# flashlight/wav2letter

Measured on AMD Instinct MI355X. Metric: utterances/sec, higher is better.
Workload: dtype f32

## Files before the change

### include/w2l_hip.h

```cpp
#ifndef W2L_HIP_H_
#define W2L_HIP_H_

#include <stddef.h>
#include <stdint.h>

#ifdef __cplusplus
extern "C" {
#endif

typedef void* w2l_stream_t;

typedef enum {
  W2L_OK = 0,
  W2L_EINVAL = 1,
  W2L_EHIP = 2,
  W2L_EUNSUPPORTED = 3
} w2l_status;

typedef enum {
  W2L_SCALE_NONE = 0,
  W2L_SCALE_INPUT_SZ = 1,
  W2L_SCALE_INPUT_SZ_SQRT = 2,
  W2L_SCALE_TARGET_SZ = 3,
  W2L_SCALE_TARGET_SZ_SQRT = 4
// ... 142 lines not shown
                                    float* dx, w2l_stream_t stream);
int w2l_tds_conv_bf16_backward_filter(const w2l_conv_desc* d, const float* x, const float* dy, float* dw, w2l_stream_t stream);
int w2l_tds_conv_bf16_backward_filter_bias(const w2l_conv_desc* d, const float* x, const float* dy, float* dw, float* dbias,
                                           w2l_stream_t stream);

typedef struct {
  uint16_t* rowMajor;
  size_t ldRows;
  uint16_t* transposed;
  size_t ldTrans;
} w2l_bf16_image_sink;
int w2l_gemm_bf16_images(int M, int N, int K, const uint16_t* A, int lda, const uint16_t* B, int ldb, float* C, int ldc,
                         const float* bias, int relu, const w2l_gemm_epilogue* epilogue, const w2l_bf16_image_sink* images,
                         const uint16_t* maskImage, size_t ldMask, float maskScale, w2l_stream_t stream);
size_t w2l_layernorm_scratch_doubles(int groups, size_t inner);
int w2l_residual_layernorm_forward(int groups, size_t inner, float* a, const float* x, float* r,
                                   float* y, const float* gammaBeta, float eps, double p,
                                   uint32_t seed, uint32_t rngStream, double* stats,
                                   float* meanRstd, w2l_stream_t stream);
int w2l_layernorm_backward(int groups, size_t inner, const float* r, const float* dy,
                           const float* gammaBeta, const float* meanRstd, float* dr,
                           float* dGammaBeta, const float* maskSrc, float* dmask, float maskScale,
                           double* sums, w2l_stream_t stream);
int w2l_residual_layernorm_forward_images(int groups, size_t inner, float* a, const float* x, float* r, float* y,
                                          const float* gammaBeta, float eps, double p, uint32_t seed, uint32_t rngStream,
                                          float* meanRstd, const w2l_bf16_image_sink* yImages, w2l_stream_t stream);
int w2l_layernorm_backward_images(int groups, size_t inner, const float* r, const float* dy, const float* gammaBeta,
                                  const float* meanRstd, float* dr, float* dGammaBeta, const float* maskSrc, float* dmask,
                                  float maskScale, double* sums, const w2l_bf16_image_sink* drImages, double imageDropP,
                                  uint32_t imageDropSeed, uint32_t imageDropStream, w2l_stream_t stream);
int w2l_dropout_inplace(float* x, size_t n, double p, uint32_t seed, uint32_t rngStream,
                        w2l_stream_t stream);
int w2l_dropout_copy(float* y, const float* x, size_t n, double p, uint32_t seed, uint32_t rngStream,
                     w2l_stream_t stream);
int w2l_mask_backward(const float* dy, const float* src, float* dx, size_t n, float scale,
                      w2l_stream_t stream);

int w2l_hexpand_forward(const float* x, float* xe, size_t rows, int H, int C, int kh, int padh, w2l_stream_t stream);
int w2l_hexpand_backward(const float* dxe, float* dx, size_t rows, int H, int C, int kh, int padh, w2l_stream_t stream);
typedef struct {
  int M, N, K, G1, G2;
  long long sam, sak, a1, a2;
  long long sbk, sbn, b1, b2;
  long long ldc, c1, c2;
  int accumulate;
  int bandMode, bandT, bandH, bandOff;
// ... 115 lines not shown
```

### wav2letter_amd/_lib.py

```python
import ctypes as C
import os

_HERE = os.path.dirname(os.path.abspath(__file__))
SO_PATH = os.environ.get("W2L_HIP_SO") or os.path.join(_HERE, "libw2l_hip.so")
_lib = None

W2L_OK, W2L_EINVAL, W2L_EHIP, W2L_EUNSUPPORTED = 0, 1, 2, 3
_ERR = {1: "W2L_EINVAL (bad shape / null pointer)", 2: "W2L_EHIP (HIP runtime error)",
        3: "W2L_EUNSUPPORTED (shape outside this build)"}


class W2LError(RuntimeError):
    pass


class W2LInvalidArgument(W2LError, ValueError):
    """mirrors the std::invalid_argument Flashlight's criteria throw"""


def _load(path):
    if not os.path.exists(path):
        raise W2LError(
            f"{path} not found: build it with `python -c 'import __graft_entry__ as g; g.build()'` "
            "or `make -C wav2letter_amd/csrc` (no CPU fallback exists)")
# ... 88 lines not shown
    w2l_gemm_bf16_ex = (_i, [_i, _i, _i, _p, _i, _i, _p, _i, _i, _p, _i, _p, _i, _p, _p])
    w2l_gemm_bf16_grouped = (_i, [_i, _i, _i, _i, _p, _i, _p, _i, _p, _i, _p, _p])
    w2l_tds_conv_bf16_image_elems = (_sz, [_p])
    w2l_tds_conv_bf16_prepare = (_i, [_p, _p, _p, _p, _p])
    w2l_tds_conv_bf16_forward = (_i, [_p, _p, _p, _p, _p, _i, _p])
    w2l_tds_conv_bf16_backward_data = (_i, [_p, _p, _p, _p, _p, _p])
    w2l_tds_conv_bf16_backward_filter = (_i, [_p, _p, _p, _p, _p])
    w2l_tds_conv_bf16_backward_filter_bias = (_i, [_p, _p, _p, _p, _p, _p])
    w2l_mfsc_spectrum = (_i, [_p, _p, _sz, _i, _i, _i, _p])
    w2l_mfsc_log_transpose = (_i, [_p, _p, _i, _i, _i, _i, _f, _p])
    w2l_weightnorm_forward = (_i, [_p, _p, _p, _p, _i, _i, _p])
    w2l_weightnorm_backward = (_i, [_p, _p, _p, _p, _p, _p, _p, _i, _i, _p])
    w2l_conv_out_len = (_i, [_i, _i, _i, _i, _i])
    w2l_conv_same_pad = (_i, [_i, _i, _i])
    w2l_conv_forward = (_i, [_p, _p, _p, _p, _p, _i, _p])
    w2l_conv_backward_data = (_i, [_p, _p, _p, _p, _i, _p])
    w2l_conv_backward_data_add = (_i, [_p, _p, _p, _p, _p, _p])
    w2l_conv_backward_filter = (_i, [_p, _p, _p, _p, _p, _p])
    w2l_layernorm_scratch_doubles = (_sz, [_i, _sz])
    w2l_residual_layernorm_forward_images = (_i, [_i, _sz, _p, _p, _p, _p, _p, _f, _d, _u32, _u32, _p, _p, _p])
    w2l_layernorm_backward_images = (_i, [_i, _sz, _p, _p, _p, _p, _p, _p, _p, _p, _f, _p, _p, _d, _u32, _u32, _p])
    w2l_residual_layernorm_forward = (_i, [_i, _sz, _p, _p, _p, _p, _p, _f, _d, _u32, _u32, _p, _p, _p])
    w2l_layernorm_backward = (_i, [_i, _sz, _p, _p, _p, _p, _p, _p, _p, _p, _f, _p, _p])
    w2l_dropout_inplace = (_i, [_p, _sz, _d, _u32, _u32, _p])
    w2l_dropout_copy = (_i, [_p, _p, _sz, _d, _u32, _u32, _p])
    w2l_linear_forward_dropout = (_i, [_i, _i, _i, _p, _p, _p, _p, _i, _d, _u32, _u32, _p])
    w2l_linear_forward_dropout_add = (_i, [_i, _i, _i, _p, _p, _p, _p, _p, _i, _d, _u32, _u32, _p])
    w2l_linear_backward_data_add = (_i, [_i, _i, _i, _p, _p, _p, _p, _p])
    w2l_mask_backward = (_i, [_p, _p, _p, _sz, _f, _p])
    w2l_hexpand_forward = (_i, [_p, _p, _sz, _i, _i, _i, _i, _p])
    w2l_hexpand_backward = (_i, [_p, _p, _sz, _i, _i, _i, _i, _p])
    w2l_bgemm_f32 = (_i, [_p, _p, _p, _p, _p])
    w2l_bgemm_bf16 = (_i, [_p, _p, _p, _p, _p])
    w2l_attn_softmax_forward = (_i, [_p, _p, _p, _i, _i, _i, _i, _i, _i, _i, _f, _p])
    w2l_attn_fused_forward = (_i, [_p, _p, _p, _p, _p, _p, _p, _p, _p, _p])
    w2l_attn_fused_backward_workspace = (_sz, [_p, _i])
    w2l_attn_fused_forward_images = (_i, [_p, _p, _p, _p, _p, _p, _p, _p, _p, _p, _p])
    w2l_attn_fused_backward_images = (_i, [_p, _p, _p, _p, _p, _p, _p, _p, _p, _p, _p, _p, _p, _p, _p, _sz, _p])
    w2l_attn_fused_backward = (_i, [_p, _p, _p, _p, _p, _p, _p, _p, _p, _p, _p, _p, _sz, _p])
    w2l_attn_key_lengths = (_i, [_p, _i, _i, _i, _p, _p])
    w2l_attn_key_lengths_full = (_i, [_p, _p, _i, _i, _i, _p, _p])
    w2l_attn_softmax_backward = (_i, [_p, _p, _p, _i, _i, _i, _i, _i, _i, _i, _f, _p])
    w2l_pool_time_forward = (_i, [_p, _p, _i, _i, _i, _i, _i, _p])
    w2l_pool_time_backward = (_i, [_p, _p, _p, _i, _i, _i, _i, _i, _p])
    w2l_axpy = (_i, [_p, _p, _sz, _f, _p])
    w2l_transpose = (_i, [_p, _p, _i, _i, _i, _p])
# ... 62 lines not shown
```

### wav2letter_amd/csrc/elementwise.hip

```cpp
#include "common.hpp"
#include "gemm.hpp"

namespace w2l {

constexpr int kEwThreads = 256;

static inline unsigned ew_grid(size_t n4) {
  size_t g = (n4 + kEwThreads - 1) / kEwThreads;
  if (g > 256 * 16) g = 256 * 16;
  if (g < 1) g = 1;
  return (unsigned)g;
}

constexpr int kLnMaxParts = 64;
constexpr size_t kLnSmall = 8192;

__device__ __forceinline__ void block_partial2(double a, double b, double* part) {
  __shared__ double sm[2][kEwThreads / 64];
#pragma unroll
  for (int off = 32; off > 0; off >>= 1) {
    a += __shfl_xor(a, off);
    b += __shfl_xor(b, off);
  }
  const int w = threadIdx.x >> 6;
  if ((threadIdx.x & 63) == 0) { sm[0][w] = a; sm[1][w] = b; }
  __syncthreads();
  if (threadIdx.x == 0) {
    double sa = 0, sb = 0;
#pragma unroll
    for (int i = 0; i < kEwThreads / 64; ++i) { sa += sm[0][i]; sb += sm[1][i]; }
    part[0] = sa;
    part[1] = sb;
  }
}
__device__ __forceinline__ void sum_parts(const double* __restrict__ part, int g, int nparts, double& a, double& b) {
  a = 0; b = 0;
  for (int i = 0; i < nparts; ++i) { a += part[2 * ((size_t)g * nparts + i)]; b += part[2 * ((size_t)g * nparts + i) + 1]; }
}

__global__ __launch_bounds__(kEwThreads) void residual_dropout_stats_k(
    float* __restrict__ a, const float* __restrict__ x, float* __restrict__ r, double* __restrict__ part,
    size_t inner, uint32_t thr, float keepScale, uint32_t seed, uint32_t stream) {
  const int g = blockIdx.y;
  const size_t base = (size_t)g * inner;
  const size_t n4 = inner >> 2;
  double s = 0, ss = 0;
  for (size_t i = (size_t)blockIdx.x * blockDim.x + threadIdx.x; i < n4; i += (size_t)gridDim.x * blockDim.x) {
    const size_t e = base + 4 * i;
    float4 av = *(const float4*)(a + e);
    float4 rv = x ? *(const float4*)(x + e) : make_float4(0.f, 0.f, 0.f, 0.f);
    if (thr) {
      av.x = keep_elem(e, seed, stream, thr) ? av.x * keepScale : 0.f;
      av.y = keep_elem(e + 1, seed, stream, thr) ? av.y * keepScale : 0.f;
      av.z = keep_elem(e + 2, seed, stream, thr) ? av.z * keepScale : 0.f;
      av.w = keep_elem(e + 3, seed, stream, thr) ? av.w * keepScale : 0.f;
      if (r != a || !x) *(float4*)(a + e) = av;
    }
    rv.x += av.x; rv.y += av.y; rv.z += av.z; rv.w += av.w;
    if (r != a || x) *(float4*)(r + e) = rv;
    const float p1 = (rv.x + rv.y) + (rv.z + rv.w);
    const float p2 = (rv.x * rv.x + rv.y * rv.y) + (rv.z * rv.z + rv.w * rv.w);
    s += (double)p1;
    ss += (double)p2;
  }
  block_partial2(s, ss, part + 2 * ((size_t)g * gridDim.x + blockIdx.x));
}

__global__ __launch_bounds__(kEwThreads) void ln_apply_k(const float* __restrict__ r, float* __restrict__ y,
                                                        const double* __restrict__ part,
                                                        float* __restrict__ meanRstd, size_t inner,
                                                        const float* __restrict__ gammaBeta, float eps) {
  const int g = blockIdx.y;
  double s1, s2;
  sum_parts(part, g, gridDim.x, s1, s2);
  const double mu = s1 / (double)inner;
  double var = s2 / (double)inner - mu * mu;
  if (var < 0) var = 0;
  const float rstd = (float)(1.0 / sqrt(var + (double)eps));
  const float muf = (float)mu;
  if (blockIdx.x == 0 && threadIdx.x == 0) { meanRstd[2 * g] = muf; meanRstd[2 * g + 1] = rstd; }
// ... 164 lines not shown
  if (threadIdx.x == 0) { meanRstd[2 * g] = muf; meanRstd[2 * g + 1] = rstd; }
  const float gam = gammaBeta[0] * rstd, bet = gammaBeta[1];
  for (size_t i = threadIdx.x; i < inner; i += kEwThreads) y[base + i] = (r[base + i] - muf) * gam + bet;
}

__global__ __launch_bounds__(kEwThreads) void ln_bwd_reduce_k(const float* __restrict__ r,
                                                             const float* __restrict__ dy,
                                                             const float* __restrict__ meanRstd,
                                                             double* __restrict__ part, size_t inner) {
  const int g = blockIdx.y;
  const float mu = meanRstd[2 * g], rstd = meanRstd[2 * g + 1];
  const size_t base = (size_t)g * inner, n4 = inner >> 2;
  double s1 = 0, s2 = 0;
  for (size_t i = (size_t)blockIdx.x * blockDim.x + threadIdx.x; i < n4; i += (size_t)gridDim.x * blockDim.x) {
    float4 rv = *(const float4*)(r + base + 4 * i);
    float4 dv = *(const float4*)(dy + base + 4 * i);
    s1 += (double)((dv.x + dv.y) + (dv.z + dv.w));
    s2 += (double)((dv.x * ((rv.x - mu) * rstd) + dv.y * ((rv.y - mu) * rstd)) +
                   (dv.z * ((rv.z - mu) * rstd) + dv.w * ((rv.w - mu) * rstd)));
  }
  block_partial2(s1, s2, part + 2 * ((size_t)g * gridDim.x + blockIdx.x));
}

__global__ __launch_bounds__(kEwThreads) void ln_bwd_apply_k(const float* __restrict__ r,
                                                            const float* __restrict__ dy,
                                                            const float* __restrict__ meanRstd,
                                                            const double* __restrict__ part,
                                                            double* __restrict__ sums,
                                                            const float* __restrict__ gammaBeta,
                                                            float* __restrict__ dr,
                                                            const float* __restrict__ maskSrc,
                                                            float* __restrict__ dmask, float maskScale,
                                                            size_t inner) {
  const int g = blockIdx.y;
  const float mu = meanRstd[2 * g], rstd = meanRstd[2 * g + 1];
  double S1, S2;
  sum_parts(part, g, gridDim.x, S1, S2);
  if (blockIdx.x == 0 && threadIdx.x == 0) { sums[2 * g] = S1; sums[2 * g + 1] = S2; }
  const float c1 = (float)(S1 / (double)inner), c2 = (float)(S2 / (double)inner);
  const float gr = gammaBeta[0] * rstd;
  const size_t base = (size_t)g * inner, n4 = inner >> 2;
  for (size_t i = (size_t)blockIdx.x * blockDim.x + threadIdx.x; i < n4; i += (size_t)gridDim.x * blockDim.x) {
    const size_t e = base + 4 * i;
    float4 rv = *(const float4*)(r + e);
    float4 dv = *(const float4*)(dy + e);
    float4 o;
    o.x = gr * (dv.x - c1 - (rv.x - mu) * rstd * c2);
    o.y = gr * (dv.y - c1 - (rv.y - mu) * rstd * c2);
    o.z = gr * (dv.z - c1 - (rv.z - mu) * rstd * c2);
    o.w = gr * (dv.w - c1 - (rv.w - mu) * rstd * c2);
    *(float4*)(dr + e) = o;
    if (dmask) {
      float4 mv = *(const float4*)(maskSrc + e);
      float4 d2;
      d2.x = mv.x > 0.f ? o.x * maskScale : 0.f;
      d2.y = mv.y > 0.f ? o.y * maskScale : 0.f;
      d2.z = mv.z > 0.f ? o.z * maskScale : 0.f;
      d2.w = mv.w > 0.f ? o.w * maskScale : 0.f;
      *(float4*)(dmask + e) = d2;
    }
  }
}

template <int NJ>
__global__ __launch_bounds__(kEwThreads) void ln_bwd_small_k(const float* __restrict__ r, const float* __restrict__ dy,
                                                            const float* __restrict__ meanRstd,
                                                            double* __restrict__ sums,
                                                            const float* __restrict__ gammaBeta,
                                                            float* __restrict__ dr,
                                                            const float* __restrict__ maskSrc,
                                                            float* __restrict__ dmask, float maskScale,
                                                            size_t inner) {
  __shared__ double bc[2];
  const int g = blockIdx.x;
  const float mu = meanRstd[2 * g], rstd = meanRstd[2 * g + 1];
  const size_t base = (size_t)g * inner;
  const int n4 = (int)(inner >> 2);
  float4 xh[NJ], dv[NJ], mvs[NJ];
  const int lastc = n4 - 1;
#pragma unroll
  for (int j = 0; j < NJ; ++j) {
// ... 424 lines not shown
    }
#undef W2L_LN_FWDW
    W2L_LAUNCH_CHECK();
    return W2L_OK;
  }
  if (inner <= kLnSmall) {
    const int nj = (int)((inner / 4 + kEwThreads - 1) / kEwThreads);
#define W2L_LN_FWD(NJ_)                                                                                                     \
  case NJ_:                                                                                                                 \
    hipLaunchKernelGGL(residual_ln_small_k<NJ_>, dim3((unsigned)groups), dim3(kEwThreads), 0, W2L_S, a, x, r, y, meanRstd,  \
                       inner, gammaBeta, eps, thr, ks, seed, rngStream);                                                    \
    break
    switch (nj) {
      W2L_LN_FWD(1); W2L_LN_FWD(2); W2L_LN_FWD(3); W2L_LN_FWD(4); W2L_LN_FWD(5); W2L_LN_FWD(6); W2L_LN_FWD(7);
      default: hipLaunchKernelGGL(residual_ln_small_k<kLnSmallV>, dim3((unsigned)groups), dim3(kEwThreads), 0, W2L_S, a, x, r, y, meanRstd,
                                  inner, gammaBeta, eps, thr, ks, seed, rngStream);
    }
#undef W2L_LN_FWD
    W2L_LAUNCH_CHECK();
    return W2L_OK;
  }
  double* part = stats + 2 * (size_t)groups;
  dim3 grid(ln_parts(inner), (unsigned)groups);
  hipLaunchKernelGGL(residual_dropout_stats_k, grid, dim3(kEwThreads), 0, W2L_S, a, x, r, part, inner, thr, ks, seed, rngStream);
  W2L_LAUNCH_CHECK();
  hipLaunchKernelGGL(ln_apply_k, grid, dim3(kEwThreads), 0, W2L_S, r, y, part, meanRstd, inner, gammaBeta, eps);
  W2L_LAUNCH_CHECK();
  return W2L_OK;
}

W2L_API int w2l_layernorm_backward(int groups, size_t inner, const float* r, const float* dy,
                                   const float* gammaBeta, const float* meanRstd, float* dr,
                                   float* dGammaBeta, const float* maskSrc, float* dmask, float maskScale,
                                   double* sums, w2l_stream_t stream) {
  if (groups <= 0 || inner == 0 || (inner & 3) || !r || !dy || !gammaBeta || !meanRstd || !dr || !sums)
    return W2L_EINVAL;
  if (inner / 4 <= 64 * (size_t)kLnWaveV && ln_wave_enabled()) {
    const int nj = (int)((inner / 4 + 63) / 64);
    const dim3 grid((unsigned)((groups + kEwThreads / 64 - 1) / (kEwThreads / 64)));
#define W2L_LN_BWDW(NJ_)                                                                                                 \
  case NJ_:                                                                                                              \
    hipLaunchKernelGGL(ln_bwd_wave_k<NJ_>, grid, dim3(kEwThreads), 0, W2L_S, groups, r, dy, meanRstd, sums, gammaBeta,   \
                       dr, maskSrc, maskSrc ? dmask : nullptr, maskScale, inner);                                        \
    break
    switch (nj) {
      W2L_LN_BWDW(1); W2L_LN_BWDW(2); W2L_LN_BWDW(3); W2L_LN_BWDW(4); W2L_LN_BWDW(5); W2L_LN_BWDW(6); W2L_LN_BWDW(7); W2L_LN_BWDW(8);
      default: hipLaunchKernelGGL(ln_bwd_wave_k<kLnWaveV>, grid, dim3(kEwThreads), 0, W2L_S, groups, r, dy, meanRstd, sums, gammaBeta,
                                  dr, maskSrc, maskSrc ? dmask : nullptr, maskScale, inner);
    }
#undef W2L_LN_BWDW
    W2L_LAUNCH_CHECK();
  } else if (inner <= kLnSmall) {
    const int nj = (int)((inner / 4 + kEwThreads - 1) / kEwThreads);
#define W2L_LN_BWD(NJ_)                                                                                                  \
  case NJ_:                                                                                                              \
    hipLaunchKernelGGL(ln_bwd_small_k<NJ_>, dim3((unsigned)groups), dim3(kEwThreads), 0, W2L_S, r, dy, meanRstd, sums,   \
                       gammaBeta, dr, maskSrc, maskSrc ? dmask : nullptr, maskScale, inner);                             \
    break
    switch (nj) {
      W2L_LN_BWD(1); W2L_LN_BWD(2); W2L_LN_BWD(3); W2L_LN_BWD(4); W2L_LN_BWD(5); W2L_LN_BWD(6); W2L_LN_BWD(7);
      default: hipLaunchKernelGGL(ln_bwd_small_k<kLnSmallV>, dim3((unsigned)groups), dim3(kEwThreads), 0, W2L_S, r, dy, meanRstd, sums,
                                  gammaBeta, dr, maskSrc, maskSrc ? dmask : nullptr, maskScale, inner);
    }
#undef W2L_LN_BWD
    W2L_LAUNCH_CHECK();
  } else {
    double* part = sums + 2 * (size_t)groups;
    dim3 grid(ln_parts(inner), (unsigned)groups);
    hipLaunchKernelGGL(ln_bwd_reduce_k, grid, dim3(kEwThreads), 0, W2L_S, r, dy, meanRstd, part, inner);
    W2L_LAUNCH_CHECK();
    hipLaunchKernelGGL(ln_bwd_apply_k, grid, dim3(kEwThreads), 0, W2L_S, r, dy, meanRstd, part, sums, gammaBeta, dr,
                       maskSrc, maskSrc ? dmask : nullptr, maskScale, inner);
    W2L_LAUNCH_CHECK();
  }
  if (dGammaBeta) {
    hipLaunchKernelGGL(ln_param_grad_k, dim3(1), dim3(1024), 0, W2L_S, sums, groups, dGammaBeta);
    W2L_LAUNCH_CHECK();
  }
  return W2L_OK;
}

__global__ __launch_bounds__(kEwThreads) void dropout_copy_k(float* __restrict__ y, const float* __restrict__ x, size_t n,
                                                            uint32_t thr, float keepScale, uint32_t seed, uint32_t stream) {
  const size_t n4 = n >> 2;
  for (size_t i = (size_t)blockIdx.x * blockDim.x + threadIdx.x; i < n4; i += (size_t)gridDim.x * blockDim.x) {
    const size_t e = 4 * i;
    float4 v = *(const float4*)(x + e);
    v.x = keep_elem(e, seed, stream, thr) ? v.x * keepScale : 0.f;
    v.y = keep_elem(e + 1, seed, stream, thr) ? v.y * keepScale : 0.f;
    v.z = keep_elem(e + 2, seed, stream, thr) ? v.z * keepScale : 0.f;
    v.w = keep_elem(e + 3, seed, stream, thr) ? v.w * keepScale : 0.f;
    *(float4*)(y + e) = v;
  }
  for (size_t e = (n4 << 2) + (size_t)blockIdx.x * blockDim.x + threadIdx.x; e < n; e += (size_t)gridDim.x * blockDim.x)
    y[e] = keep_elem(e, seed, stream, thr) ? x[e] * keepScale : 0.f;
}

W2L_API int w2l_dropout_copy(float* y, const float* x, size_t n, double p, uint32_t seed, uint32_t rngStream,
                             w2l_stream_t stream) {
  if (!x || !y || ((((uintptr_t)x) | ((uintptr_t)y)) & 15)) return W2L_EINVAL;
  const uint32_t thr = dropout_threshold(p);
  if (!n) return W2L_OK;
// ... 172 lines not shown
```

### wav2letter_amd/csrc/host/net.cpp

```cpp
#include <algorithm>
#include <cmath>
#include <cstring>
#include <sstream>

#include "w2l_host.hpp"

namespace w2l {

std::string Act::str() const {
  std::ostringstream os;
  os << "(";
  for (int i = 0; i < 4; ++i) {
    os << (i ? "," : "");
    if (d[i].f.size() == 1 && d[i].f[0].kind == F_TIME) os << "T";
    else if (d[i].f.size() == 1 && d[i].f[0].kind == F_BATCH) os << "B";
    else os << d[i].size();
  }
  os << ") phys[" << B << "][" << T << "][" << F << "]";
  return os.str();
}

static constexpr int kSymT = 1000003, kSymB = 1000033;

Act actInput(int B, int T, int nFeat) {
// ... 349 lines not shown
    if (!rides) check(w2l_colsum(g, b.g(cx), (size_t)M, bl.out, cx.stream), "bwd b");
  }
  void backward(Ctx& cx, float* ar, const float* x, const BfImage& xImg, const float* dy, const BfImage& dyImg, const float* addend, float* dx, double p) {
    const bool mixed = cx.bf16;
    const bool rides2 = mixed ? lin2BiasRides(cx) : biasWithWeight, rides1 = mixed ? bl1.biasRides(xImg, w1->g(cx), b1->g(cx)) : biasWithWeight;
    const float sc = (float)(1.0 / (1.0 - p));
    float *u = ar + uOff, *du = ar + duOff;
    weightGrad(cx, ar, bl2, u, uImg, dy, dyImg, *w2, *b2, rides2);
    if (!mixed) {
      check(w2l_linear_backward_data(M, hidden, in, dy, w2->w(cx), du, 0, u, sc, cx.stream), "lin2 bwd x");
    } else if (!(uOnlyImages && bl2.backwardDataImages(cx, ar, dyImg, rides1 ? nullptr : du, &duImg, uImg, sc))) {
      if (uOnlyImages) throw std::runtime_error(tag("u was kept as images only, but the image-writing backward-data product refused"));
      bl2.backwardData(cx, ar, dyImg, du, u, sc, nullptr, 0);
      duImg.convert(cx, ar, du, tag("du images").c_str());
    }
    weightGrad(cx, ar, bl1, x, xImg, du, duImg, *w1, *b1, rides1);
    if (mixed) bl1.backwardData(cx, ar, duImg, dx, nullptr, 1.f, addend, 0);
    else check(w2l_linear_backward_data_add(M, in, hidden, du, w1->w(cx), addend, dx, cx.stream), "lin1 bwd x");
  }
};

constexpr size_t kLnImageElems = (size_t)1 << 22;
static bool lnForward(Ctx& cx, float* ar, int groups, size_t inner, float* a, const float* x, float* r, float* y, const float* gb, double p,
                      uint32_t seed, uint32_t stream, double* stats, float* mr, const BfImage* img, const char* what) {
  if (img && img->rows == groups && (size_t)img->cols == inner && (size_t)groups * inner <= kLnImageElems) {
    const w2l_bf16_image_sink k = img->sink(cx, ar);
    const int st = w2l_residual_layernorm_forward_images(groups, inner, a, x, r, y, gb, 1e-5f, p, seed, stream, mr, &k, cx.stream);
    if (st == W2L_OK) return true;
    if (st != W2L_EUNSUPPORTED) w2lCheck(st, what);
  }
  w2lCheck(w2l_residual_layernorm_forward(groups, inner, a, x, r, y, gb, 1e-5f, p, seed, stream, stats, mr, cx.stream), what);
  return false;
}
static bool lnBackward(Ctx& cx, float* ar, int groups, size_t inner, const float* r, const float* dy, const float* gb, const float* mr, float* dr,
                       float* dgb, const float* maskSrc, float* dmask, float maskScale, double* sums, const BfImage* img, double imgP,
                       uint32_t imgSeed, uint32_t imgStream, const char* what) {
  if (img && img->rows == groups && (size_t)img->cols == inner && (size_t)groups * inner <= kLnImageElems) {
    const w2l_bf16_image_sink k = img->sink(cx, ar);
    const int st = w2l_layernorm_backward_images(groups, inner, r, dy, gb, mr, dr, dgb, maskSrc, dmask, maskScale, sums, &k, imgP, imgSeed,
                                                 imgStream, cx.stream);
    if (st == W2L_OK) return true;
    if (st != W2L_EUNSUPPORTED) w2lCheck(st, what);
  }
  w2lCheck(w2l_layernorm_backward(groups, inner, r, dy, gb, mr, dr, dgb, maskSrc, dmask, maskScale, sums, cx.stream), what);
  return false;
}

struct WNState {
  bool on = false;
  P v, g;
  size_t wOff = 0, dwOff = 0, normOff = 0, dotOff = 0;
  int K = 0, N = 0;
};

// ... 313 lines not shown
    w2lCheck(w2l_glu_forward(x, y, M, half, c.stream), "glu fwd");
  }
  void backward(Ctx& c, float* arena, const float* dy, float*& dx, bool) override {
    dx = arena + dxOff;
    w2lCheck(w2l_glu_backward(xSaved, dy, dx, M, half, c.stream), "glu bwd");
  }
};

class TDSLayer : public Layer {
 public:
  int c, kw, h, l, l2, rPad;
  double p;
  bool lnTime;
  P wc, bc, gb1, w1, b1, w2, b2, gb2;
  w2l_conv_desc d{};
  int B = 0, T = 0, M = 0, groups = 0;
  size_t inner = 0, n = 0;
  size_t aOff, r1Off, y1Off, vOff, outOff, st1Off, mr1Off, st2Off, mr2Off;
  size_t dsOff, dy1Off, dr1Off, daOff, dxOff;
  const float* xSaved = nullptr;
  FeedForward ff;
  BfImage y1Img, dvImg;
  size_t convImgElems = 0, convImgFOff = 0, convImgBOff = 0;

  std::string name() const override { return "TDSBlock"; }
  void registerParams(std::vector<ParamInfo>& t) override {
    ParamInfo q;
    q = ParamInfo(); q.name = "tds.conv.w"; q.numel = (size_t)kw * c * c; q.refShape = {kw, 1, c, c}; q.kind = 1;
    q.kw = kw; q.cin = c; q.cout = c; q.initBound = std::sqrt(1.0 / ((double)c * kw)); addParam(t, q, wc);
    q = ParamInfo(); q.name = "tds.conv.b"; q.numel = c; q.refShape = {1, 1, c, 1}; q.initBound = std::sqrt(1.0 / ((double)c * kw)); addParam(t, q, bc);
    q = ParamInfo(); q.name = "tds.ln1.weight+bias"; q.numel = 2; q.refShape = {1}; q.kind = 3; addParam(t, q, gb1);
    q = ParamInfo(); q.name = "tds.lin1.w"; q.numel = (size_t)l * l2; q.refShape = {l2, l}; q.kind = 2; q.cin = l; q.cout = l2;
    q.initBound = std::sqrt(1.0 / (double)l); addParam(t, q, w1);
    q = ParamInfo(); q.name = "tds.lin1.b"; q.numel = l2; q.refShape = {l2}; q.initBound = std::sqrt(1.0 / (double)l); addParam(t, q, b1);
    q = ParamInfo(); q.name = "tds.lin2.w"; q.numel = (size_t)l2 * l; q.refShape = {l, l2}; q.kind = 2; q.cin = l2; q.cout = l;
    q.initBound = std::sqrt(1.0 / (double)l2); addParam(t, q, w2);
    q = ParamInfo(); q.name = "tds.lin2.b"; q.numel = l; q.refShape = {l}; q.initBound = std::sqrt(1.0 / (double)l2); addParam(t, q, b2);
    q = ParamInfo(); q.name = "tds.ln2.weight+bias"; q.numel = 2; q.refShape = {1}; q.kind = 3; addParam(t, q, gb2);
  }
  Act plan(const Act& in, Planner& pl) override {
    int H;
    requireConvLayout(in, c, "TDSBlock", H);
    if (H != h) throw std::invalid_argument("TDSBlock: expected H=" + std::to_string(h) + ", input " + in.str());
    int pL, pR;
    if (rPad < 0) { pL = pR = samePad(in.T, kw, 1); }
    else { if (rPad > kw - 1) throw std::invalid_argument("TDSBlock: invalid right padding"); pR = rPad; pL = kw - 1 - rPad; }
    d = {in.B, in.T, h, c, c, kw, 1, pL, pR};
    if (w2l_conv_out_len(in.T, kw, 1, pL, pR) != in.T) throw std::invalid_argument("TDSBlock: conv must preserve T (odd kw)");
    B = in.B; T = in.T; M = B * T; n = in.numel();
    groups = lnTime ? B : B * T;
    inner = n / groups;
    if (inner % 4) throw std::invalid_argument("TDSBlock: LayerNorm size must be a multiple of 4");
    aOff = pl.alloc(n); r1Off = pl.alloc(n); y1Off = pl.alloc(n); vOff = pl.alloc(n); outOff = pl.alloc(n);
    st1Off = pl.alloc(2 * w2l_layernorm_scratch_doubles(groups, inner)); mr1Off = pl.alloc(2 * (size_t)groups);
    st2Off = pl.alloc(2 * w2l_layernorm_scratch_doubles(groups, inner)); mr2Off = pl.alloc(2 * (size_t)groups);
    dsOff = pl.alloc(n); dy1Off = pl.alloc(n); dr1Off = pl.alloc(n); daOff = pl.alloc(n); dxOff = pl.alloc(n);
    ff.joinInLin2 = l2 % 32 == 0;
    ff.biasWithWeight = true;
    ff.plan(pl, "tds", M, l, l2, w1, b1, w2, b2);
    y1Img.plan(pl, M, l, true); dvImg.plan(pl, M, l);
    convImgElems = h % 16 == 0 ? w2l_tds_conv_bf16_image_elems(&d) : 0;
    if (convImgElems) { convImgFOff = pl.allocBf16(convImgElems); convImgBOff = pl.allocBf16(convImgElems); }
    return in;
  }
  void forward(Ctx& cx, float* ar, const float* x, float*& y) override {
    hipStream_t s = cx.stream;
    const double pd = cx.train ? p : 0.0;
    xSaved = x;
    float *a = ar + aOff, *r1 = ar + r1Off, *y1 = ar + y1Off, *v = ar + vOff, *out = ar + outOff;
    if (cx.bf16 && convImgElems) {
      w2lCheck(w2l_tds_conv_bf16_prepare(&d, wc.w(cx), bfp(ar, convImgFOff), bfp(ar, convImgBOff), s), "tds conv images");
      w2lCheck(w2l_tds_conv_bf16_forward(&d, x, bfp(ar, convImgFOff), bc.w(cx), a, 1, s), "tds conv bf16");
    } else {
      w2lCheck(w2l_conv_forward(&d, x, wc.w(cx), bc.w(cx), a, 1, s), "tds conv");
    }
    const bool y1Images = lnForward(cx, ar, groups, inner, a, x, r1, y1, gb1.w(cx), pd, cx.seed, rngStream, (double*)(ar + st1Off), ar + mr1Off,
                                    cx.bf16 ? &y1Img : nullptr, "tds ln1");
    if (cx.bf16) {
      const w2l_bf16_convert_desc wd[3] = {y1Img.desc(ar, y1), ff.bl1.w.desc(ar, w1.w(cx)), ff.bl2.w.desc(ar, w2.w(cx))};
      w2lCheck(w2l_bf16_convert_multi(y1Images ? 2 : 3, wd + (y1Images ? 1 : 0), s), "tds y1 + weight images");
      if (!y1Images) y1Img.ensureOnes(cx, ar);
    }
    const bool joined = ff.forward(cx, ar, y1, y1Img, v, pd, rngStream + 1);
    w2lCheck(w2l_residual_layernorm_forward(groups, inner, v, joined ? nullptr : y1, v, out, gb2.w(cx), 1e-5f, joined ? 0.0 : pd,
                                            joined ? 0 : cx.seed, joined ? 0 : rngStream + 2, (double*)(ar + st2Off), ar + mr2Off, s), "tds ln2");
    y = out;
  }
  void backward(Ctx& cx, float* ar, const float* dy, float*& dx, bool needDx) override {
    hipStream_t s = cx.stream;
    const double pd = cx.train ? p : 0.0;
    const float sc = (float)(1.0 / (1.0 - pd));
    float *a = ar + aOff, *y1 = ar + y1Off, *v = ar + vOff;
    float *ds = ar + dsOff, *dy1 = ar + dy1Off, *dr1 = ar + dr1Off, *da = ar + daOff;
    const bool rides2 = cx.bf16 && ff.lin2BiasRides(cx);
    const bool maskInConvert = pd > 0 && rides2;
    const bool dvImages = lnBackward(cx, ar, groups, inner, v, dy, gb2.w(cx), ar + mr2Off, ds, gb2.g(cx), nullptr, nullptr, 1.f,
                                     (double*)(ar + st2Off), cx.bf16 && (pd == 0 || maskInConvert) ? &dvImg : nullptr, pd, cx.seed,
                                     rngStream + 2, "tds ln2 bwd");
    const float* dv = ds;
    if (pd > 0 && !maskInConvert) {
      w2lCheck(w2l_dropout_copy(dy1, ds, n, pd, cx.seed, rngStream + 2, s), "tds do2 bwd");
      dv = dy1;
    }
    if (cx.bf16 && !dvImages) {
      if (maskInConvert) dvImg.convertDropout(cx, ar, ds, pd, cx.seed, rngStream + 2, "tds dv images (masked)");
      else dvImg.convert(cx, ar, dv, "tds dv images");
    }
    ff.backward(cx, ar, y1, y1Img, dv, dvImg, ds, dy1, pd);
    w2lCheck(w2l_layernorm_backward(groups, inner, ar + r1Off, dy1, gb1.w(cx), ar + mr1Off, dr1, gb1.g(cx), a, da, sc,
                                    (double*)(ar + st1Off), s), "tds ln1 bwd");
    if (cx.bf16 && convImgElems) {
      w2lCheck(w2l_tds_conv_bf16_backward_filter_bias(&d, xSaved, da, wc.g(cx), bc.g(cx), s), "tds conv bwd filter + bias bf16");
      if (needDx) {
        dx = ar + dxOff;
        w2lCheck(w2l_tds_conv_bf16_backward_data(&d, da, bfp(ar, convImgBOff), dr1, dx, s), "tds conv bwd data bf16");
      }
      return;
    }
    w2lCheck(w2l_conv_backward_filter(&d, xSaved, da, wc.g(cx), bc.g(cx), s), "tds conv bwd filter");
    if (needDx) {
      dx = ar + dxOff;
      w2lCheck(w2l_conv_backward_data_add(&d, da, wc.w(cx), dr1, dx, s), "tds conv bwd data");
    }
  }
};

class PoolTimeLayer : public Layer {
 public:
  int w = 1, stride = 1;
  int B = 0, T = 0, To = 0, F = 0;
  size_t yOff = 0, dxOff = 0;
  const float* xSaved = nullptr;
  std::string name() const override { return "Pool2D"; }
// ... 673 lines not shown
```

### wav2letter_amd/ops.py

```python
import ctypes as C

import torch

from . import _lib
from ._lib import ConvDesc, check


def _s():
    return torch.cuda.current_stream().cuda_stream


def _p(t):
    return t.data_ptr() if t is not None else None


def gemm(A, B, a_kcontig=True, b_kcontig=False, bias=None, relu=False, splitk=1):
    M, K = (A.shape if a_kcontig else A.shape[::-1])
    N = B.shape[0] if b_kcontig else B.shape[1]
    Cm = torch.empty(M, N, device=A.device, dtype=torch.float32)
    check(_lib.lib().w2l_gemm_f32(M, N, K, _p(A), A.stride(0), int(a_kcontig), _p(B), B.stride(0), int(b_kcontig),
                                  _p(Cm), N, _p(bias), int(relu), splitk, _s()), "gemm")
    return Cm


# ... 70 lines not shown
def _ln_scratch(groups, inner):
    return int(_lib.lib().w2l_layernorm_scratch_doubles(groups, inner))


def residual_layernorm_forward(a, x, gamma_beta, groups, eps=1e-5, p=0.0, seed=0, stream_id=0):
    inner = a.numel() // groups
    r = torch.empty_like(a)
    y = torch.empty_like(a)
    stats = torch.empty(_ln_scratch(groups, inner), device=a.device, dtype=torch.float64)
    mr = torch.empty(2 * groups, device=a.device, dtype=torch.float32)
    check(_lib.lib().w2l_residual_layernorm_forward(groups, inner, _p(a), _p(x), _p(r), _p(y), _p(gamma_beta), eps,
                                                    p, seed, stream_id, _p(stats), _p(mr), _s()), "res_ln_fwd")
    return y, r, mr


def layernorm_backward(r, dy, gamma_beta, mean_rstd, groups, mask_src=None, mask_scale=1.0):
    inner = r.numel() // groups
    dr = torch.empty_like(r)
    dgb = torch.empty(2, device=r.device, dtype=torch.float32)
    dmask = torch.empty_like(r) if mask_src is not None else None
    sums = torch.empty(_ln_scratch(groups, inner), device=r.device, dtype=torch.float64)
    check(_lib.lib().w2l_layernorm_backward(groups, inner, _p(r), _p(dy), _p(gamma_beta), _p(mean_rstd), _p(dr),
                                            _p(dgb), _p(mask_src), _p(dmask), mask_scale, _p(sums), _s()), "ln_bwd")
    return dr, dgb, dmask


def linear_forward_dropout(x, w, bias, relu, p, seed, stream_id):
    M, K = x.shape
    N = w.shape[1]
    y = torch.empty(M, N, device=x.device, dtype=torch.float32)
    check(_lib.lib().w2l_linear_forward_dropout(M, K, N, _p(x), _p(w), _p(bias), _p(y), int(relu), p, seed, stream_id, _s()), "linear_forward_dropout")
    return y


def linear_forward_dropout_add(x, w, bias, add, relu, p, seed, stream_id):
    M, K = x.shape
    N = w.shape[1]
    y = torch.empty(M, N, device=x.device, dtype=torch.float32)
    check(_lib.lib().w2l_linear_forward_dropout_add(M, K, N, _p(x), _p(w), _p(bias), _p(add), _p(y), int(relu), p, seed, stream_id, _s()),
          "linear_forward_dropout_add")
    return y


def linear_backward_data_add(dy, w, add):
    M, N = dy.shape
    K = w.shape[0]
# ... 154 lines not shown
```

Measured before the change: 328.6.

## Fuse dropout mask bits and recomputed dropout into TDS layernorm backward

```diff
diff --git a/include/w2l_hip.h b/include/w2l_hip.h
--- a/include/w2l_hip.h
+++ b/include/w2l_hip.h
@@ -188,6 +188,16 @@
                            const float* gammaBeta, const float* meanRstd, float* dr,
                            float* dGammaBeta, const float* maskSrc, float* dmask, float maskScale,
                            double* sums, w2l_stream_t stream);
+size_t w2l_layernorm_mask_bytes(int groups, size_t inner);
+int w2l_residual_layernorm_forward_mask(int groups, size_t inner, const float* a, const float* x, float* r, float* y,
+                                        const float* gammaBeta, float eps, double p, uint32_t seed, uint32_t rngStream,
+                                        double* stats, float* meanRstd, uint8_t* mask, w2l_stream_t stream);
+int w2l_layernorm_backward_mask(int groups, size_t inner, const float* r, const float* dy, const float* gammaBeta,
+                                const float* meanRstd, float* dr, float* dGammaBeta, const uint8_t* mask, float* dmask,
+                                float maskScale, double* sums, w2l_stream_t stream);
+int w2l_layernorm_backward_dropout(int groups, size_t inner, const float* r, const float* dy, const float* gammaBeta,
+                                   const float* meanRstd, float* dr, float* dGammaBeta, float* dmask, double p, uint32_t seed,
+                                   uint32_t rngStream, double* sums, w2l_stream_t stream);
 int w2l_residual_layernorm_forward_images(int groups, size_t inner, float* a, const float* x, float* r, float* y,
                                           const float* gammaBeta, float eps, double p, uint32_t seed, uint32_t rngStream,
                                           float* meanRstd, const w2l_bf16_image_sink* yImages, w2l_stream_t stream);
diff --git a/wav2letter_amd/_lib.py b/wav2letter_amd/_lib.py
--- a/wav2letter_amd/_lib.py
+++ b/wav2letter_amd/_lib.py
@@ -134,6 +134,10 @@
     w2l_layernorm_backward_images = (_i, [_i, _sz, _p, _p, _p, _p, _p, _p, _p, _p, _f, _p, _p, _d, _u32, _u32, _p])
     w2l_residual_layernorm_forward = (_i, [_i, _sz, _p, _p, _p, _p, _p, _f, _d, _u32, _u32, _p, _p, _p])
     w2l_layernorm_backward = (_i, [_i, _sz, _p, _p, _p, _p, _p, _p, _p, _p, _f, _p, _p])
+    w2l_layernorm_mask_bytes = (_sz, [_i, _sz])
+    w2l_residual_layernorm_forward_mask = (_i, [_i, _sz, _p, _p, _p, _p, _p, _f, _d, _u32, _u32, _p, _p, _p, _p])
+    w2l_layernorm_backward_mask = (_i, [_i, _sz, _p, _p, _p, _p, _p, _p, _p, _p, _f, _p, _p])
+    w2l_layernorm_backward_dropout = (_i, [_i, _sz, _p, _p, _p, _p, _p, _p, _p, _d, _u32, _u32, _p, _p])
     w2l_dropout_inplace = (_i, [_p, _sz, _d, _u32, _u32, _p])
     w2l_dropout_copy = (_i, [_p, _p, _sz, _d, _u32, _u32, _p])
     w2l_linear_forward_dropout = (_i, [_i, _i, _i, _p, _p, _p, _p, _i, _d, _u32, _u32, _p])
diff --git a/wav2letter_amd/csrc/elementwise.hip b/wav2letter_amd/csrc/elementwise.hip
--- a/wav2letter_amd/csrc/elementwise.hip
+++ b/wav2letter_amd/csrc/elementwise.hip
@@ -1,3 +1,4 @@
+#include <type_traits>
 #include "common.hpp"
 #include "gemm.hpp"
 
@@ -38,9 +39,11 @@
   for (int i = 0; i < nparts; ++i) { a += part[2 * ((size_t)g * nparts + i)]; b += part[2 * ((size_t)g * nparts + i) + 1]; }
 }
 
+template <bool MASK>
 __global__ __launch_bounds__(kEwThreads) void residual_dropout_stats_k(
-    float* __restrict__ a, const float* __restrict__ x, float* __restrict__ r, double* __restrict__ part,
-    size_t inner, uint32_t thr, float keepScale, uint32_t seed, uint32_t stream) {
+    std::conditional_t<MASK, const float, float>* __restrict__ a, const float* __restrict__ x, float* __restrict__ r,
+    double* __restrict__ part, uint8_t* __restrict__ mask, size_t inner, uint32_t thr, float keepScale, uint32_t seed,
+    uint32_t stream) {
   const int g = blockIdx.y;
   const size_t base = (size_t)g * inner;
   const size_t n4 = inner >> 2;
@@ -54,8 +57,11 @@
       av.y = keep_elem(e + 1, seed, stream, thr) ? av.y * keepScale : 0.f;
       av.z = keep_elem(e + 2, seed, stream, thr) ? av.z * keepScale : 0.f;
       av.w = keep_elem(e + 3, seed, stream, thr) ? av.w * keepScale : 0.f;
-      if (r != a || !x) *(float4*)(a + e) = av;
-    }
+      if constexpr (!MASK)
+        if (r != a || !x) *(float4*)(a + e) = av;
+    }
+    if constexpr (MASK)
+      mask[e >> 2] = (uint8_t)((av.x > 0.f ? 1 : 0) | (av.y > 0.f ? 2 : 0) | (av.z > 0.f ? 4 : 0) | (av.w > 0.f ? 8 : 0));
     rv.x += av.x; rv.y += av.y; rv.z += av.z; rv.w += av.w;
     if (r != a || x) *(float4*)(r + e) = rv;
     const float p1 = (rv.x + rv.y) + (rv.z + rv.w);
@@ -266,6 +272,9 @@
   block_partial2(s1, s2, part + 2 * ((size_t)g * gridDim.x + blockIdx.x));
 }
 
+enum { LN_MASK_SRC = 0, LN_MASK_BITS = 1, LN_MASK_HASH = 2 };
+struct LnHash { uint32_t thr, seed, stream; };
+template <int MODE>
 __global__ __launch_bounds__(kEwThreads) void ln_bwd_apply_k(const float* __restrict__ r,
                                                             const float* __restrict__ dy,
                                                             const float* __restrict__ meanRstd,
@@ -274,13 +283,35 @@
                                                             const float* __restrict__ gammaBeta,
                                                             float* __restrict__ dr,
                                                             const float* __restrict__ maskSrc,
+                                                            const uint8_t* __restrict__ maskBits, LnHash hash,
                                                             float* __restrict__ dmask, float maskScale,
-                                                            size_t inner) {
+                                                            size_t inner, float* __restrict__ dGammaBeta) {
   const int g = blockIdx.y;
   const float mu = meanRstd[2 * g], rstd = meanRstd[2 * g + 1];
   double S1, S2;
   sum_parts(part, g, gridDim.x, S1, S2);
   if (blockIdx.x == 0 && threadIdx.x == 0) { sums[2 * g] = S1; sums[2 * g + 1] = S2; }
+  if (dGammaBeta && blockIdx.x == 0 && g == 0) {
+    __shared__ double r1[kEwThreads], r2[kEwThreads];
+    const int tid = threadIdx.x;
+    double a1 = 0, a2 = 0;
+    if (tid < (int)gridDim.y) {
+      double t1, t2;
+      sum_parts(part, tid, gridDim.x, t1, t2);
+      a1 += t1; a2 += t2;
+    }
+    r1[tid] = a1;
+    r2[tid] = a2;
+    __syncthreads();
+    for (int off = kEwThreads / 2; off > 0; off >>= 1) {
+      if (tid < off) { r1[tid] += r1[tid + off]; r2[tid] += r2[tid + off]; }
+      __syncthreads();
+    }
+    if (tid == 0) {
+      dGammaBeta[0] = (float)r2[0];
+      dGammaBeta[1] = (float)r1[0];
+    }
+  }
   const float c1 = (float)(S1 / (double)inner), c2 = (float)(S2 / (double)inner);
   const float gr = gammaBeta[0] * rstd;
   const size_t base = (size_t)g * inner, n4 = inner >> 2;
@@ -294,13 +325,23 @@
     o.z = gr * (dv.z - c1 - (rv.z - mu) * rstd * c2);
     o.w = gr * (dv.w - c1 - (rv.w - mu) * rstd * c2);
     *(float4*)(dr + e) = o;
-    if (dmask) {
-      float4 mv = *(const float4*)(maskSrc + e);
+    if (MODE != LN_MASK_SRC || dmask) {
+      bool k0, k1, k2, k3;
+      if constexpr (MODE == LN_MASK_SRC) {
+        const float4 mv = *(const float4*)(maskSrc + e);
+        k0 = mv.x > 0.f; k1 = mv.y > 0.f; k2 = mv.z > 0.f; k3 = mv.w > 0.f;
+      } else if constexpr (MODE == LN_MASK_BITS) {
+        const unsigned m = maskBits[e >> 2];
+        k0 = m & 1; k1 = m & 2; k2 = m & 4; k3 = m & 8;
+      } else {
+        k0 = keep_elem(e, hash.seed, hash.stream, hash.thr); k1 = keep_elem(e + 1, hash.seed, hash.stream, hash.thr);
+        k2 = keep_elem(e + 2, hash.seed, hash.stream, hash.thr); k3 = keep_elem(e + 3, hash.seed, hash.stream, hash.thr);
+      }
       float4 d2;
-      d2.x = mv.x > 0.f ? o.x * maskScale : 0.f;
-      d2.y = mv.y > 0.f ? o.y * maskScale : 0.f;
-      d2.z = mv.z > 0.f ? o.z * maskScale : 0.f;
-      d2.w = mv.w > 0.f ? o.w * maskScale : 0.f;
+      d2.x = k0 ? o.x * maskScale : 0.f;
+      d2.y = k1 ? o.y * maskScale : 0.f;
+      d2.z = k2 ? o.z * maskScale : 0.f;
+      d2.w = k3 ? o.w * maskScale : 0.f;
       *(float4*)(dmask + e) = d2;
     }
   }
@@ -771,10 +812,52 @@
   }
   double* part = stats + 2 * (size_t)groups;
   dim3 grid(ln_parts(inner), (unsigned)groups);
-  hipLaunchKernelGGL(residual_dropout_stats_k, grid, dim3(kEwThreads), 0, W2L_S, a, x, r, part, inner, thr, ks, seed, rngStream);
+  hipLaunchKernelGGL(residual_dropout_stats_k<false>, grid, dim3(kEwThreads), 0, W2L_S, a, x, r, part, (uint8_t*)nullptr, inner, thr, ks,
+                     seed, rngStream);
   W2L_LAUNCH_CHECK();
   hipLaunchKernelGGL(ln_apply_k, grid, dim3(kEwThreads), 0, W2L_S, r, y, part, meanRstd, inner, gammaBeta, eps);
   W2L_LAUNCH_CHECK();
+  return W2L_OK;
+}
+
+W2L_API size_t w2l_layernorm_mask_bytes(int groups, size_t inner) {
+  if (groups <= 0 || inner <= kLnSmall || (inner & 3)) return 0;
+  return (size_t)groups * (inner >> 2);
+}
+
+W2L_API int w2l_residual_layernorm_forward_mask(int groups, size_t inner, const float* a, const float* x, float* r, float* y,
+                                                const float* gammaBeta, float eps, double p, uint32_t seed, uint32_t rngStream,
+                                                double* stats, float* meanRstd, uint8_t* mask, w2l_stream_t stream) {
+  if (groups <= 0 || inner == 0 || !a || !r || r == a || !y || !gammaBeta || !stats || !meanRstd || !mask) return W2L_EINVAL;
+  if (!w2l_layernorm_mask_bytes(groups, inner)) return W2L_EUNSUPPORTED;
+  const uint32_t thr = dropout_threshold(p);
+  const float ks = (float)(1.0 / (1.0 - p));
+  double* part = stats + 2 * (size_t)groups;
+  dim3 grid(ln_parts(inner), (unsigned)groups);
+  hipLaunchKernelGGL(residual_dropout_stats_k<true>, grid, dim3(kEwThreads), 0, W2L_S, a, x, r, part, mask, inner, thr, ks, seed,
+                     rngStream);
+  W2L_LAUNCH_CHECK();
+  hipLaunchKernelGGL(ln_apply_k, grid, dim3(kEwThreads), 0, W2L_S, r, y, part, meanRstd, inner, gammaBeta, eps);
+  W2L_LAUNCH_CHECK();
+  return W2L_OK;
+}
+
+template <int MODE>
+static int ln_backward_two_pass(int groups, size_t inner, const float* r, const float* dy, const float* gammaBeta, const float* meanRstd,
+                                float* dr, float* dGammaBeta, const float* maskSrc, const uint8_t* maskBits, LnHash hash, float* dmask,
+                                float maskScale, double* sums, hipStream_t stream) {
+  double* part = sums + 2 * (size_t)groups;
+  dim3 grid(ln_parts(inner), (unsigned)groups);
+  hipLaunchKernelGGL(ln_bwd_reduce_k, grid, dim3(kEwThreads), 0, stream, r, dy, meanRstd, part, inner);
+  W2L_LAUNCH_CHECK();
+  const bool fold = dGammaBeta && groups <= kEwThreads;
+  hipLaunchKernelGGL(ln_bwd_apply_k<MODE>, grid, dim3(kEwThreads), 0, stream, r, dy, meanRstd, part, sums, gammaBeta, dr, maskSrc,
+                     maskBits, hash, dmask, maskScale, inner, fold ? dGammaBeta : nullptr);
+  W2L_LAUNCH_CHECK();
+  if (dGammaBeta && !fold) {
+    hipLaunchKernelGGL(ln_param_grad_k, dim3(1), dim3(1024), 0, stream, sums, groups, dGammaBeta);
+    W2L_LAUNCH_CHECK();
+  }
   return W2L_OK;
 }
 
@@ -814,19 +897,34 @@
 #undef W2L_LN_BWD
     W2L_LAUNCH_CHECK();
   } else {
-    double* part = sums + 2 * (size_t)groups;
-    dim3 grid(ln_parts(inner), (unsigned)groups);
-    hipLaunchKernelGGL(ln_bwd_reduce_k, grid, dim3(kEwThreads), 0, W2L_S, r, dy, meanRstd, part, inner);
-    W2L_LAUNCH_CHECK();
-    hipLaunchKernelGGL(ln_bwd_apply_k, grid, dim3(kEwThreads), 0, W2L_S, r, dy, meanRstd, part, sums, gammaBeta, dr,
-                       maskSrc, maskSrc ? dmask : nullptr, maskScale, inner);
-    W2L_LAUNCH_CHECK();
+    return ln_backward_two_pass<LN_MASK_SRC>(groups, inner, r, dy, gammaBeta, meanRstd, dr, dGammaBeta, maskSrc, nullptr, LnHash{},
+                                             maskSrc ? dmask : nullptr, maskScale, sums, W2L_S);
   }
   if (dGammaBeta) {
     hipLaunchKernelGGL(ln_param_grad_k, dim3(1), dim3(1024), 0, W2L_S, sums, groups, dGammaBeta);
     W2L_LAUNCH_CHECK();
   }
   return W2L_OK;
+}
+
+W2L_API int w2l_layernorm_backward_mask(int groups, size_t inner, const float* r, const float* dy, const float* gammaBeta,
+                                        const float* meanRstd, float* dr, float* dGammaBeta, const uint8_t* mask, float* dmask,
+                                        float maskScale, double* sums, w2l_stream_t stream) {
+  if (groups <= 0 || inner == 0 || (inner & 3) || !r || !dy || !gammaBeta || !meanRstd || !dr || !mask || !dmask || !sums)
+    return W2L_EINVAL;
+  if (!w2l_layernorm_mask_bytes(groups, inner)) return W2L_EUNSUPPORTED;
+  return ln_backward_two_pass<LN_MASK_BITS>(groups, inner, r, dy, gammaBeta, meanRstd, dr, dGammaBeta, nullptr, mask, LnHash{}, dmask,
+                                            maskScale, sums, W2L_S);
+}
+
+W2L_API int w2l_layernorm_backward_dropout(int groups, size_t inner, const float* r, const float* dy, const float* gammaBeta,
+                                           const float* meanRstd, float* dr, float* dGammaBeta, float* dmask, double p,
+                                           uint32_t seed, uint32_t rngStream, double* sums, w2l_stream_t stream) {
+  if (groups <= 0 || inner == 0 || (inner & 3) || !r || !dy || !gammaBeta || !meanRstd || !dr || !dmask || !sums) return W2L_EINVAL;
+  if (inner <= kLnSmall) return W2L_EUNSUPPORTED;
+  return ln_backward_two_pass<LN_MASK_HASH>(groups, inner, r, dy, gammaBeta, meanRstd, dr, dGammaBeta, nullptr, nullptr,
+                                            LnHash{dropout_threshold(p), seed, rngStream}, dmask, (float)(1.0 / (1.0 - p)), sums,
+                                            W2L_S);
 }
 
 __global__ __launch_bounds__(kEwThreads) void dropout_copy_k(float* __restrict__ y, const float* __restrict__ x, size_t n,
diff --git a/wav2letter_amd/csrc/host/net.cpp b/wav2letter_amd/csrc/host/net.cpp
--- a/wav2letter_amd/csrc/host/net.cpp
+++ b/wav2letter_amd/csrc/host/net.cpp
@@ -395,14 +395,16 @@
 
 constexpr size_t kLnImageElems = (size_t)1 << 22;
 static bool lnForward(Ctx& cx, float* ar, int groups, size_t inner, float* a, const float* x, float* r, float* y, const float* gb, double p,
-                      uint32_t seed, uint32_t stream, double* stats, float* mr, const BfImage* img, const char* what) {
+                      uint32_t seed, uint32_t stream, double* stats, float* mr, const BfImage* img, const char* what,
+                      uint8_t* mask = nullptr) {
   if (img && img->rows == groups && (size_t)img->cols == inner && (size_t)groups * inner <= kLnImageElems) {
     const w2l_bf16_image_sink k = img->sink(cx, ar);
     const int st = w2l_residual_layernorm_forward_images(groups, inner, a, x, r, y, gb, 1e-5f, p, seed, stream, mr, &k, cx.stream);
     if (st == W2L_OK) return true;
     if (st != W2L_EUNSUPPORTED) w2lCheck(st, what);
   }
-  w2lCheck(w2l_residual_layernorm_forward(groups, inner, a, x, r, y, gb, 1e-5f, p, seed, stream, stats, mr, cx.stream), what);
+  if (mask) w2lCheck(w2l_residual_layernorm_forward_mask(groups, inner, a, x, r, y, gb, 1e-5f, p, seed, stream, stats, mr, mask, cx.stream), what);
+  else w2lCheck(w2l_residual_layernorm_forward(groups, inner, a, x, r, y, gb, 1e-5f, p, seed, stream, stats, mr, cx.stream), what);
   return false;
 }
 static bool lnBackward(Ctx& cx, float* ar, int groups, size_t inner, const float* r, const float* dy, const float* gb, const float* mr, float* dr,
@@ -762,6 +764,8 @@
   FeedForward ff;
   BfImage y1Img, dvImg;
   size_t convImgElems = 0, convImgFOff = 0, convImgBOff = 0;
+  size_t maskBytes = 0, maskOff = 0;
+  bool maskWritten = false;
 
   std::string name() const override { return "TDSBlock"; }
   void registerParams(std::vector<ParamInfo>& t) override {
@@ -801,6 +805,8 @@
     y1Img.plan(pl, M, l, true); dvImg.plan(pl, M, l);
     convImgElems = h % 16 == 0 ? w2l_tds_conv_bf16_image_elems(&d) : 0;
     if (convImgElems) { convImgFOff = pl.allocBf16(convImgElems); convImgBOff = pl.allocBf16(convImgElems); }
+    maskBytes = w2l_layernorm_mask_bytes(groups, inner);
+    if (maskBytes) maskOff = pl.alloc((maskBytes + 3) / 4);
     return in;
   }
   void forward(Ctx& cx, float* ar, const float* x, float*& y) override {
@@ -815,7 +821,8 @@
       w2lCheck(w2l_conv_forward(&d, x, wc.w(cx), bc.w(cx), a, 1, s), "tds conv");
     }
     const bool y1Images = lnForward(cx, ar, groups, inner, a, x, r1, y1, gb1.w(cx), pd, cx.seed, rngStream, (double*)(ar + st1Off), ar + mr1Off,
-                                    cx.bf16 ? &y1Img : nullptr, "tds ln1");
+                                    cx.bf16 ? &y1Img : nullptr, "tds ln1", maskBytes ? (uint8_t*)(ar + maskOff) : nullptr);
+    maskWritten = maskBytes && !y1Images;
     if (cx.bf16) {
       const w2l_bf16_convert_desc wd[3] = {y1Img.desc(ar, y1), ff.bl1.w.desc(ar, w1.w(cx)), ff.bl2.w.desc(ar, w2.w(cx))};
       w2lCheck(w2l_bf16_convert_multi(y1Images ? 2 : 3, wd + (y1Images ? 1 : 0), s), "tds y1 + weight images");
@@ -834,11 +841,21 @@
     float *ds = ar + dsOff, *dy1 = ar + dy1Off, *dr1 = ar + dr1Off, *da = ar + daOff;
     const bool rides2 = cx.bf16 && ff.lin2BiasRides(cx);
     const bool maskInConvert = pd > 0 && rides2;
-    const bool dvImages = lnBackward(cx, ar, groups, inner, v, dy, gb2.w(cx), ar + mr2Off, ds, gb2.g(cx), nullptr, nullptr, 1.f,
-                                     (double*)(ar + st2Off), cx.bf16 && (pd == 0 || maskInConvert) ? &dvImg : nullptr, pd, cx.seed,
-                                     rngStream + 2, "tds ln2 bwd");
+    bool dvWritten = false, dvImages = false;
+    if (!cx.bf16 && pd > 0) {
+      const int st = w2l_layernorm_backward_dropout(groups, inner, v, dy, gb2.w(cx), ar + mr2Off, ds, gb2.g(cx), dy1, pd, cx.seed,
+                                                    rngStream + 2, (double*)(ar + st2Off), s);
+      if (st != W2L_EUNSUPPORTED) w2lCheck(st, "tds ln2 bwd + do2 bwd");
+      dvWritten = st == W2L_OK;
+    }
+    if (!dvWritten)
+      dvImages = lnBackward(cx, ar, groups, inner, v, dy, gb2.w(cx), ar + mr2Off, ds, gb2.g(cx), nullptr, nullptr, 1.f,
+                            (double*)(ar + st2Off), cx.bf16 && (pd == 0 || maskInConvert) ? &dvImg : nullptr, pd, cx.seed,
+                            rngStream + 2, "tds ln2 bwd");
     const float* dv = ds;
-    if (pd > 0 && !maskInConvert) {
+    if (dvWritten) {
+      dv = dy1;
+    } else if (pd > 0 && !maskInConvert) {
       w2lCheck(w2l_dropout_copy(dy1, ds, n, pd, cx.seed, rngStream + 2, s), "tds do2 bwd");
       dv = dy1;
     }
@@ -847,8 +864,12 @@
       else dvImg.convert(cx, ar, dv, "tds dv images");
     }
     ff.backward(cx, ar, y1, y1Img, dv, dvImg, ds, dy1, pd);
-    w2lCheck(w2l_layernorm_backward(groups, inner, ar + r1Off, dy1, gb1.w(cx), ar + mr1Off, dr1, gb1.g(cx), a, da, sc,
-                                    (double*)(ar + st1Off), s), "tds ln1 bwd");
+    if (maskWritten)
+      w2lCheck(w2l_layernorm_backward_mask(groups, inner, ar + r1Off, dy1, gb1.w(cx), ar + mr1Off, dr1, gb1.g(cx),
+                                           (const uint8_t*)(ar + maskOff), da, sc, (double*)(ar + st1Off), s), "tds ln1 bwd");
+    else
+      w2lCheck(w2l_layernorm_backward(groups, inner, ar + r1Off, dy1, gb1.w(cx), ar + mr1Off, dr1, gb1.g(cx), a, da, sc,
+                                      (double*)(ar + st1Off), s), "tds ln1 bwd");
     if (cx.bf16 && convImgElems) {
       w2lCheck(w2l_tds_conv_bf16_backward_filter_bias(&d, xSaved, da, wc.g(cx), bc.g(cx), s), "tds conv bwd filter + bias bf16");
       if (needDx) {
diff --git a/wav2letter_amd/ops.py b/wav2letter_amd/ops.py
--- a/wav2letter_amd/ops.py
+++ b/wav2letter_amd/ops.py
@@ -116,6 +116,44 @@
     sums = torch.empty(_ln_scratch(groups, inner), device=r.device, dtype=torch.float64)
     check(_lib.lib().w2l_layernorm_backward(groups, inner, _p(r), _p(dy), _p(gamma_beta), _p(mean_rstd), _p(dr),
                                             _p(dgb), _p(mask_src), _p(dmask), mask_scale, _p(sums), _s()), "ln_bwd")
+    return dr, dgb, dmask
+
+
+def layernorm_mask_bytes(groups, inner):
+    return int(_lib.lib().w2l_layernorm_mask_bytes(groups, inner))
+
+
+def residual_layernorm_forward_mask(a, x, gamma_beta, groups, eps=1e-5, p=0.0, seed=0, stream_id=0):
+    inner = a.numel() // groups
+    r = torch.empty_like(a)
+    y = torch.empty_like(a)
+    stats = torch.empty(_ln_scratch(groups, inner), device=a.device, dtype=torch.float64)
+    mr = torch.empty(2 * groups, device=a.device, dtype=torch.float32)
+    mask = torch.empty(max(layernorm_mask_bytes(groups, inner), 1), device=a.device, dtype=torch.uint8)
+    check(_lib.lib().w2l_residual_layernorm_forward_mask(groups, inner, _p(a), _p(x), _p(r), _p(y), _p(gamma_beta), eps,
+                                                         p, seed, stream_id, _p(stats), _p(mr), _p(mask), _s()), "res_ln_fwd_mask")
+    return y, r, mr, mask
+
+
+def layernorm_backward_mask(r, dy, gamma_beta, mean_rstd, groups, mask, mask_scale=1.0):
+    inner = r.numel() // groups
+    dr = torch.empty_like(r)
+    dgb = torch.empty(2, device=r.device, dtype=torch.float32)
+    dmask = torch.empty_like(r)
+    sums = torch.empty(_ln_scratch(groups, inner), device=r.device, dtype=torch.float64)
+    check(_lib.lib().w2l_layernorm_backward_mask(groups, inner, _p(r), _p(dy), _p(gamma_beta), _p(mean_rstd), _p(dr),
+                                                 _p(dgb), _p(mask), _p(dmask), mask_scale, _p(sums), _s()), "ln_bwd_mask")
+    return dr, dgb, dmask
+
+
+def layernorm_backward_dropout(r, dy, gamma_beta, mean_rstd, groups, p, seed, stream_id):
+    inner = r.numel() // groups
+    dr = torch.empty_like(r)
+    dgb = torch.empty(2, device=r.device, dtype=torch.float32)
+    dmask = torch.empty_like(r)
+    sums = torch.empty(_ln_scratch(groups, inner), device=r.device, dtype=torch.float64)
+    check(_lib.lib().w2l_layernorm_backward_dropout(groups, inner, _p(r), _p(dy), _p(gamma_beta), _p(mean_rstd), _p(dr),
+                                                    _p(dgb), _p(dmask), p, seed, stream_id, _p(sums), _s()), "ln_bwd_dropout")
     return dr, dgb, dmask
 
 
```

Result: no change. 330.4, median of 6 (+0.5%).
